# goldbricklemon/uplift-upsample-3dhpe

Hardware: AMD Instinct MI355X
Metric: pose-sequences/sec (higher is better)
Workload: dtype f16x3 (f32 operands split into f16 hi/lo, 3 MFMA passes, f32 accumulate); 1 GPU; config/h36m_351.json forward, N=71 tokens (receptive field 351), J=17, batch 128/GPU, s_in=5, seeded Keras-default weights; global_batch=128, parallelism=batch-sharded x1, hipgraph=True, concurrent_half_batches=False, batches_in_flight=8

## Files before the change

uplift-upsample-3dhpe_amd/csrc/uu3d_commit.inc:

```
namespace {

struct Packer {
    std::vector<float> buf;
    std::vector<std::pair<size_t, size_t>> dense;
    size_t alloc(size_t n) {
        size_t off = align_up(buf.size(), 64);
        buf.resize(off + n, 0.f);
        return off;
    }
    size_t alloc_dense(size_t n) { const size_t off = alloc(n); dense.emplace_back(off, n); return off; }
};

const float* W(const uu3d_model* m, const std::string& name) {
    auto it = m->index.find(name);
    return it == m->index.end() ? nullptr : m->weights[it->second].host.data();
}

void pack_dense_t(std::vector<float>& buf, size_t off, const float* w, int K, int N, int Kp, int n0) {
    for (int k = 0; k < K; ++k)
        for (int n = 0; n < N; ++n) buf[off + (size_t)(n0 + n) * Kp + k] = w[(size_t)k * N + n];
}

}

// ... 165 lines not shown
        };
        auto add_qkv = [&](TcBuild& tb, const std::string& p) {
            std::vector<float> Wk, b, bf; qkv_of(p, Wk, b);
            tb.stages.push_back(folded(Wk, b, W(m, p + "/norm1/gamma"), W(m, p + "/norm1/beta"), dt, 3 * dt, bf));
            for (int n = 0; n < dt; ++n) bf[n] *= tc_qscale;
            std::copy_n(bf.begin(), 3 * dt, P.buf.begin() + tb.p_off + TCP_BQKV);
        };
        auto add_proj = [&](TcBuild& tb, const std::string& p) {
            const float* w = W(m, p + "/attn/projection/kernel");
            tb.stages.push_back(TcStage{std::vector<float>(w, w + (size_t)dt * dt), dt, dt, 0, true});
            std::copy_n(W(m, p + "/attn/projection/bias"), dt, P.buf.begin() + tb.p_off + TCP_BP);
        };
        auto add_fc1 = [&](TcBuild& tb, const std::string& p) {
            const float* w = W(m, p + "/mlp/fc1/kernel"); const float* b = W(m, p + "/mlp/fc1/bias");
            std::vector<float> bf;
            tb.stages.push_back(folded(std::vector<float>(w, w + (size_t)dt * ht), std::vector<float>(b, b + ht), W(m, p + "/norm2/gamma"), W(m, p + "/norm2/beta"), dt, ht, bf));
            std::copy_n(bf.begin(), ht, P.buf.begin() + tb.p_off + TCP_B1);
        };
        auto add_fc2 = [&](TcBuild& tb, const std::string& p) {
            const float* w = W(m, p + "/mlp/fc2/kernel");
            for (int half = 0; half < 2; ++half) tb.stages.push_back(TcStage{std::vector<float>(w, w + (size_t)ht * dt), ht, dt, half * dt, false});
            std::copy_n(W(m, p + "/mlp/fc2/bias"), dt, P.buf.begin() + tb.p_off + TCP_B2);
        };
        { TcBuild tb{TC_QKV, P.alloc(TCP_FLOATS), {}}; add_qkv(tb, block_name(false, 0)); tcb.push_back(std::move(tb)); }
        for (int i = 0; i < c.temporal_depth; ++i) {
            const bool last = i + 1 == c.temporal_depth;
            TcBuild tb{TC_PROJ | TC_MLP | (last ? (c.num_strided > 0 ? TC_QKV | TC_PE : 0) : TC_QKV), P.alloc(TCP_FLOATS), {}};
            add_proj(tb, block_name(false, i)); add_fc1(tb, block_name(false, i)); add_fc2(tb, block_name(false, i));
            if (!last) add_qkv(tb, block_name(false, i + 1)); else if (c.num_strided > 0) add_qkv(tb, block_name(true, 0));
            tcb.push_back(std::move(tb));
        }
        if (c.num_strided > 0) {
            TcBuild tb{TC_PROJ | TC_FC1_PLANES, P.alloc(TCP_FLOATS), {}};
            add_proj(tb, block_name(true, 0)); add_fc1(tb, block_name(true, 0));
            tcb.push_back(std::move(tb));
        }
    }

    if (m->arena_floats < P.buf.size()) {
        if (m->arena) HIPCHK(m, hipFree(m->arena));
        m->arena = nullptr;
        HIPCHK(m, hipMalloc((void**)&m->arena, P.buf.size() * sizeof(float)));
        m->arena_floats = P.buf.size();
    }
    HIPCHK(m, hipMemcpyAsync(m->arena, P.buf.data(), P.buf.size() * sizeof(float), hipMemcpyHostToDevice, stream));
    HIPCHK(m, hipStreamSynchronize(stream));
    if (c.precision == UU3D_PREC_F16X3) {
        std::vector<_Float16> hb(64, (_Float16)0.f);
        m->hplanes.clear();
        for (auto& d : P.dense) {
            const size_t hi = align_up(hb.size(), 64); hb.resize(hi + d.second);
// ... 144 lines not shown
```

uplift-upsample-3dhpe_amd/csrc/uu3d_forward.inc:

```

namespace {
struct Workspace {
    float *S, *X, *QKV, *O, *Hb, *XA, *XB, *slab, *mslab;
    unsigned char* tc_scratch;
    int* frame_list;
    float2* stats;
    size_t slab_floats;
    size_t bytes;
};
Workspace carve(const uu3d_model* m, int B, char* base) {
    const uu3d_config& c = m->cfg;
    const size_t rows = (size_t)B * c.num_frames;
    const size_t rows_s = (size_t)B * (c.num_strided > 1 ? std::max(m->L[1], 1) : 1);
    size_t off = 0;
    auto take = [&](size_t n) { size_t o = off; off = align_up(off + n, 256); return o; };
    Workspace w{};
    const size_t oS = take(rows * c.num_keypoints * c.d_spatial * 4);
    const size_t oX = take(rows * c.d_temporal * 4);
    const size_t oQ = take((rows + 128) * 3 * c.d_temporal * 4);
    const size_t oO = take((rows + 32) * c.d_temporal * 4);
    const size_t oH = take((rows + 32) * c.h_temporal * 4);
    const size_t oA = take(rows * c.d_temporal * 4);
    const size_t oB = take(rows_s * c.d_temporal * 4);
    const size_t oT = take(rows * sizeof(float2));
// ... 243 lines not shown
            else gemm_tile<64, 64>(al, Bt, M, N, Kp, 1, KT, ep);
        } else {
            EpSlab es{slab, ldslab, (size_t)M * ldslab};
            gemm_tile<64, 64>(al, Bt, M, N, Kp, slices, kps, es);
            hipLaunchKernelGGL(splitk_reduce_kernel<EP>, dim3((M * N + 255) / 256), dim3(256), 0, stream,
                               slab, slices, (size_t)M * ldslab, M, N, ldslab, ep);
        }
        end();
    }

    bool mlpf_ok(int M, const BlockDev& b) const {
        return !m->sw.no_mlpf && b.w2_mf != 0 && panel_ok(M, m->cfg.h_temporal, m->cfg.d_temporal, b.w1_pf);
    }
    void mlp_fused(const char* name, const _Float16* Af, const BlockDev& b, int M, float* mslab) {
        if (skip_mask() & 8) return;
        const int mt = (M + 127) / 128, S = MLPF_SLICES;
        begin(name, "mlp_fused", 4.0 * M * (double)m->cfg.d_temporal * m->cfg.h_temporal, 4.0 * ((double)M * 384 + 2.0 * 384 * 768 + 3.0 * M * 384));
        allow_lds<mlp_fused_h3_kernel>(PANEL_LDS_TOTAL);
        hipLaunchKernelGGL(mlp_fused_h3_kernel, dim3(8 * S, ((mt * S + 7) / 8 + S - 1) / S), dim3(256), PANEL_LDS_TOTAL, stream,
                           Af, m->harena + b.w1_pf, m->harena + b.w2_mf, b.b1, mslab, M, mt);
        end();
    }
    void tchain(const char* name, const uu3d_model::TcLaunch& t, int M, const _Float16* Of, float* X, float* XA, const float* pe, int period,
                _Float16* Q, _Float16* H, unsigned char* scratch) {
        if (skip_mask() & 128) return;
        const int mt = (M + 63) / 64;
        TChainArgs a{};
        a.M = M; a.m_tiles = mt; a.period = period; a.qscale = attn_qscale();
        a.Of = Of; a.X = X; a.XA = XA; a.pe = pe; a.W = m->harena + t.w_off; a.P = m->arena + t.p_off; a.Q = Q; a.H = H; a.scratch = scratch;
        const double cols = ((t.flags & TC_PROJ) ? 384.0 : 0.0) + ((t.flags & TC_MLP) ? 1536.0 : 0.0) + ((t.flags & TC_FC1_PLANES) ? 768.0 : 0.0) + ((t.flags & TC_QKV) ? 1152.0 : 0.0);
        begin(name, "tchain", 2.0 * M * 384.0 * cols, 4.0 * (384.0 * cols + 2.0 * M * 384.0 + ((t.flags & TC_QKV) ? M * 1152.0 : 0.0) + ((t.flags & TC_FC1_PLANES) ? M * 768.0 : 0.0)));
#define UU3D_T16_LAUNCH(F) case F: { allow_lds<tchain16_kernel<F>>(T16_LDS_TOTAL); \
            hipLaunchKernelGGL(tchain16_kernel<F>, dim3(mt), dim3(512), T16_LDS_TOTAL, stream, a); } break;
        switch (t.flags) {
            UU3D_T16_LAUNCH(TC_QKV)
            UU3D_T16_LAUNCH(TC_PROJ | TC_MLP | TC_QKV)
            UU3D_T16_LAUNCH(TC_PROJ | TC_MLP | TC_QKV | TC_PE)
            UU3D_T16_LAUNCH(TC_PROJ | TC_MLP)
            UU3D_T16_LAUNCH(TC_PROJ | TC_FC1_PLANES)
            default: status = UU3D_ERR_UNSUPPORTED; m->err = "temporal chain: unknown stage set"; break;
        }
#undef UU3D_T16_LAUNCH
        end();
    }
    void ln_res_split_frag(const char* name, float* x, int M, const float* bias2, const float* mslab, float* xa, const float* pe, int period,
                           const float* g, const float* b, _Float16* Af) {
        if (skip_mask() & 64) return;
        begin(name, "ln_split_frag", 0.0, 4.0 * (double)M * 384 * (xa ? 8 : 7));
        hipLaunchKernelGGL((ln_res_split_frag_kernel<24, 8>), dim3((M + 7) / 8), dim3(128), 0, stream, x, 384, M, 1e-5f, bias2, mslab, xa, pe, period, g, b, Af);
        end();
    }

    bool wt_ok(const float* Bt, int K) const {
        return precision == UU3D_PREC_F16X3 && !m->sw.no_wt && (K % 16) == 0 && m->hplanes.count((size_t)(Bt - m->arena)) != 0;
    }
    template <class AL, class EP>
    void gemm_wt(const char* name, const AL& al, const float* Bt, int M, int N, int K, const EP& ep, double extra_bytes = 0) {
        const int Kp = round_up(K, 32), slices = Kp / 16;
        const auto it = m->hplanes.find((size_t)(Bt - m->arena));
        const _Float16* Bh = m->harena + it->second.first; const _Float16* Bl = m->harena + it->second.second;
        const int mt = (M + 31) / 32, nt = (N + 31) / 32;
// ... 125 lines not shown
constexpr int kFewRows = 512;

struct Forward {
    uu3d_model* const m;
    Launcher Lh;
    const Workspace w;
    const uu3d_config c;
    const uint8_t* const mask;
    const int B;
    float* const full_out; float* const central_out; float* const* const attn_out;
    const bool part_body, part_tail;

    const int N = c.num_frames, J = c.num_keypoints, dt = c.d_temporal, ht = c.h_temporal, M = B * N;
    const bool has_h1 = c.full_output && c.temporal_depth > 0;
    const bool planes = (c.precision == UU3D_PREC_F16X3) && (dt % 32 == 0) && (ht % 32 == 0) && !m->sw.no_planes;
    const bool chain = Lh.throughput && planes && m->sw.tchain_mode != 0 && (m->sw.tchain_mode == 1 || (M + 127) / 128 >= m->sw.tchain_min_tiles) && !m->tchain.empty() && M >= 1024 &&
                       (Lh.attn_is_h3(N, true) || (m->sw.tchain_short && Lh.attn_h3_any(N))) && (c.num_strided == 0 || m->L[0] == N) && (double)M * 1152 * 4.0 < 4.0e9 &&
                       attn_out == nullptr;
    _Float16* const Ph = reinterpret_cast<_Float16*>(w.O);
    _Float16* const Hh = reinterpret_cast<_Float16*>(w.Hb);
    const BlockDev* pend = nullptr;
    float* xa = w.XA;
    char nm[48];

    void tokens_from_frames(const FramesIn& frames) {
        Lh.begin("frames_to_tokens", "frames_to_tokens", 0.0, 4.0 * 3.0 * M * dt);
        hipLaunchKernelGGL(frames_to_tokens_kernel, dim3((unsigned)(((size_t)M * (dt / 4) + 255) / 256)), dim3(256), 0, Lh.stream,
                           frames.features, frames.num_rows, frames.rows, mask, m->token, m->pe_t, (long)M, N, dt, w.X);
        Lh.end();
    }
    void spatial(const float* kp2d) {
        spatial_stage(Lh, c, kp2d, M, mask, w.frame_list, w.S, true, EpSpatialToTemporal{w.X, m->s2t_b, dt, mask, m->token, m->pe_t, N});
    }

    const _Float16* block_head(const char* tag, int i, const BlockDev& b, float* x, int L, const uint8_t* kmask, const BlockDev* prev, bool fuse_mlp) {
        const int Mr = B * L;
        auto name = [&](const char* what) { snprintf(nm, sizeof nm, "%s%d.%s", tag, i + 1, what); return nm; };
        _Float16* const Pl = Ph + (size_t)Mr * dt; _Float16* const Hl = Hh + (size_t)Mr * ht;
        const bool qsplit = Lh.attn_is_h3(L, planes);
        _Float16* const Qh = reinterpret_cast<_Float16*>(w.QKV); _Float16* const Ql = Qh + (size_t)Mr * 3 * dt;
        const EpBiasSplitQ ep_qs{Qh, Ql, b.bqkv, 3 * dt, dt, Lh.attn_qscale()};
        const bool few = planes && Mr <= kFewRows && Lh.wt_ok(b.wqkv_t, dt) && Lh.wt_ok(b.w1_t, dt);
        auto maps = [&]() {
            if (attn_out != nullptr && tag[0] == 't' && attn_out[i] != nullptr) {
                Lh.begin(name("attn_maps"), "attn_probs", 2.0 * B * (double)c.num_heads * L * L * kDH, 4.0 * B * (double)c.num_heads * L * L);
                const size_t lds = (size_t)L * (kDH + 1) * sizeof(float);
// ... 43 lines not shown
        }
        if (mlp_panel) {
            if (!ln2_done) Lh.ln_split_frag(name("ln2_split"), x, Mr, b.ln2_g, b.ln2_b, Ph);
            if (fuse_mlp) return Ph;
            Lh.gemm_panel(name("ln_fc1"), Ph, b.w1_pf, b.b1, Mr, ht, PanelEpBiasReluSplit{Hh, Hl, ht});
        } else {
            Lh.row_stats(name("stats2"), x, dt, Mr, w.stats);
            ALoadLayerNorm al{x, w.stats, b.ln2_g, b.ln2_b, dt, Mr, dt};
            if (planes) { EpBiasReluSplit ep{Hh, Hl, b.b1, ht}; Lh.gemm(name("ln_fc1"), al, b.w1_t, Mr, ht, dt, ep); }
            else { EpBiasRelu ep{w.Hb, b.b1, ht}; Lh.gemm(name("ln_fc1"), al, b.w1_t, Mr, ht, dt, ep); }
        }
        return nullptr;
    }

    void temporal_chain() {
        _Float16* const Q = reinterpret_cast<_Float16*>(w.QKV);
        Lh.tchain("t1.ln_qkv", m->tchain[0], M, nullptr, w.X, nullptr, nullptr, 1, Q, nullptr, w.tc_scratch);
        for (int i = 0; i < c.temporal_depth; ++i) {
            const bool masked = c.has_strided_input && i < c.first_strided_token_attention_layer;
            snprintf(nm, sizeof nm, "t%d.attn", i + 1);
            Lh.attn(nm, w.QKV, B, N, masked ? mask : nullptr, w.O, (size_t)M * dt, true, true);
            const bool to_strided = i + 1 == c.temporal_depth && c.num_strided > 0;
            snprintf(nm, sizeof nm, "t%d.chain", i + 1);
            Lh.tchain(nm, m->tchain[i + 1], M, Ph, w.X, to_strided ? w.XA : nullptr, to_strided ? m->sblocks[0].pe : nullptr, N, Q, nullptr, w.tc_scratch);
        }
    }
    void temporal_blocks() {
        for (int i = 0; i < c.temporal_depth; ++i) {
            const BlockDev& b = m->tblocks[i];
            const bool masked = c.has_strided_input && i < c.first_strided_token_attention_layer;
            const bool last = (i + 1 == c.temporal_depth);
            const bool fuse = planes && Lh.mlpf_ok(M, b) && (last ? (c.num_strided > 0 && Lh.panel_ok(M, 3 * dt, dt, m->sblocks[0].wqkv_pf))
                                                                  : Lh.panel_ok(M, 3 * dt, dt, m->tblocks[i + 1].wqkv_pf));
            const _Float16* const a2 = block_head("t", i, b, w.X, N, masked ? mask : nullptr, pend, fuse);
            pend = nullptr;
            if (fuse) {
                snprintf(nm, sizeof nm, "t%d.mlp", i + 1);
                Lh.mlp_fused(nm, a2, b, M, w.mslab);
                pend = &b;
                continue;
            }
            const bool to_strided = last && c.num_strided > 0;
            EpBiasResidual ep_fc2{w.X, b.b2, dt, to_strided ? w.XA : nullptr, to_strided ? m->sblocks[0].pe : nullptr, N};
            snprintf(nm, sizeof nm, "t%d.fc2_res", i + 1);
            if (planes) { GLoadPlain gl{Hh, Hh + (size_t)M * ht, ht, M}; Lh.gemm_g(nm, gl, b.w2_t, M, dt, ht, ep_fc2, 4.0 * M * dt); }
            else { ALoadPlain al{w.Hb, ht, M, ht}; Lh.gemm(nm, al, b.w2_t, M, dt, ht, ep_fc2, 4.0 * M * dt); }
        }
    }
    void head1() {
        if (!has_h1) return;
        ALoadPlain al{w.X, dt, M, dt}; EpBias ep{full_out, m->h1_b, 3 * J};
        Lh.gemm("head1", al, m->h1_wt, M, 3 * J, dt, ep);
    }
    void strided_blocks() {
        float* xb = w.XB;
        const _Float16* const hzero = m->harena;
        if (c.temporal_depth == 0 && c.num_strided > 0) {
            Lh.begin("s1.add_pe", "add_pe", 0.0, 12.0 * M * dt);
            hipLaunchKernelGGL(add_period_kernel, dim3((unsigned)(((size_t)M * dt / 4 + 255) / 256)), dim3(256), 0, Lh.stream, w.X, m->sblocks[0].pe, M, dt, N, w.XA);
            Lh.end();
        }
        for (int i = 0; i < c.num_strided; ++i) {
            const BlockDev& b = m->sblocks[i];
            const int Li = m->L[i], Lo = m->L[i + 1], Mi = B * Li, Mo = B * Lo;
            if (((skip_mask() & 256) || part_body) && i >= 1) continue;
            if (((skip_mask() & 512) || part_tail) && i == 0) { std::swap(xa, xb); xb = w.XA; continue; }
            const int lo = (c.strides[i] > 1 && c.pad_left[i] == 0) ? 1 : 0;
            const EpConvResidual ep_conv{xb, b.b2, dt, xa, Li, Lo, c.strides[i], lo,
                                         (i + 1 < c.num_strided) ? m->sblocks[i + 1].pe : nullptr};
            const bool smask = c.temporal_depth == 0 && c.has_strided_input && i < c.first_strided_token_attention_layer;
            if (chain && i == 0) {
                Lh.attn("s1.attn", w.QKV, B, Li, nullptr, w.O, (size_t)Mi * dt, true, true);
                Lh.tchain("s1.chain", m->tchain[c.temporal_depth + 1], Mi, Ph, nullptr, xa, nullptr, 1, nullptr, Hh, w.tc_scratch);
            } else
            block_head("s", i, b, xa, Li, smask ? mask : nullptr, i == 0 ? pend : nullptr, false);
            if (i == 0) head1();
            snprintf(nm, sizeof nm, "s%d.conv_res", i + 1);
            if (planes) { GLoadConv3 gl{Hh, Hh + (size_t)Mi * ht, hzero, ht, Li, Lo, c.strides[i], c.pad_left[i], Mo};
                          Lh.gemm_g(nm, gl, b.w2_t, Mo, dt, 3 * ht, ep_conv, 4.0 * Mo * dt); }
            else { ALoadConv3 al{w.Hb, ht, Li, Lo, c.strides[i], c.pad_left[i], Mo, 3 * ht};
                   Lh.gemm(nm, al, b.w2_t, Mo, dt, 3 * ht, ep_conv, 4.0 * Mo * dt); }
            std::swap(xa, xb);
            if (i == 0) xb = w.XA;
        }
    }
    void head2() {
        ALoadPlain al{c.num_strided > 0 ? xa : w.X + (size_t)(N / 2) * dt, c.num_strided > 0 ? dt : N * dt, B, dt};
        EpBias ep{central_out, m->h2_b, 3 * J};
        Lh.gemm("head2", al, m->h2_wt, B, 3 * J, dt, ep);
    }
    void range_check() {
        if (c.precision != UU3D_PREC_F16X3) return;
        Lh.begin("range_check", "range_check", 0.0, 4.0 * ((has_h1 ? (double)M * 3 * J : 0.0) + (double)B * 3 * J));
        hipLaunchKernelGGL(range_check_kernel, dim3(256), dim3(256), 0, Lh.stream, has_h1 ? full_out : central_out, has_h1 ? (long)M * 3 * J : 0L,
                           central_out, (long)B * 3 * J, m->d_range);
        Lh.end();
    }
};

int forward_impl(uu3d_model* m, const float* kp2d, const FramesIn* frames, const uint8_t* mask, int32_t B, float* full_out,
                 float* central_out, float* const* attn_out, void* workspace, size_t workspace_bytes, int32_t schedule, void* stream_) {
    if (!m) return UU3D_ERR_INVALID_ARGUMENT;
    const bool exact_f32 = (schedule & UU3D_SCHEDULE_EXACT_F32) != 0;
    schedule &= ~UU3D_SCHEDULE_EXACT_F32;
#ifdef UU3D_TIMING_BUILD
    const bool parts_ok = process_switches().timing_parts;
#else
    constexpr bool parts_ok = false;
#endif
    const bool part_body = parts_ok && (schedule & 0x200) != 0, part_tail = parts_ok && (schedule & 0x400) != 0;
    if (parts_ok) schedule &= ~0x600;
    if (schedule != UU3D_SCHEDULE_LATENCY && schedule != UU3D_SCHEDULE_THROUGHPUT) return fail(m, UU3D_ERR_INVALID_ARGUMENT, "schedule must be UU3D_SCHEDULE_LATENCY or UU3D_SCHEDULE_THROUGHPUT");
    if (!m->committed) return fail(m, UU3D_ERR_NOT_READY, "uu3d_commit_weights has not been called");
    if ((!kp2d && !frames) || !central_out || !workspace || B < 1) return fail(m, UU3D_ERR_INVALID_ARGUMENT, "null buffer or batch < 1");
    if (frames != nullptr) {
// ... 106 lines not shown
```

uplift-upsample-3dhpe_amd/csrc/uu3d_gemm.h:

```cpp
#pragma once
#include "uu3d_dropout.h"
#include <hip/hip_runtime.h>
#include <stdint.h>

namespace uu3d {

typedef float f32x4 __attribute__((ext_vector_type(4)));
typedef float f32x16 __attribute__((ext_vector_type(16)));

static constexpr int GEMM_BK = 32;
static constexpr int GEMM_LD = 36;

__host__ __device__ inline constexpr size_t gemm_lds_bytes(int BM, int BN) {
    return (size_t)2 * (BM + BN) * GEMM_LD * sizeof(float);
}

struct ALoadPlain {
    const float* __restrict__ A;
    int lda, M, K;
    struct Ctx { const float* p; };
    struct Raw { f32x4 x; };
    __device__ __forceinline__ Ctx prep(int row) const {
        Ctx c; c.p = A + (size_t)min(row, M - 1) * lda; return c;
    }
// ... 50 lines not shown
    }
    __device__ __forceinline__ Raw issue(const Ctx& c, int k) const {
        const int kc = min(k, K - 4);
        const int j = kc / C;
        const int cc = kc - j * C;
        const int src = c.t0 + j;
        Raw r;
        r.ok = (src >= 0) & (src < L_in) & (k < K);
        const int srcc = min(max(src, 0), L_in - 1);
        r.x = *reinterpret_cast<const f32x4*>(Hin + (size_t)(c.base_row + srcc) * C + cc);
        return r;
    }
    __device__ __forceinline__ f32x4 finish(const Ctx&, int, const Raw& r) const {
        return r.ok ? r.x : (f32x4){0.f, 0.f, 0.f, 0.f};
    }
};

struct EpBias {
    float* __restrict__ out; const float* __restrict__ bias; int ldo;
    __device__ __forceinline__ float2 colv(int col) const { return make_float2(bias[col], 0.f); }
    __device__ __forceinline__ float2 pre(int, int) const { return make_float2(0.f, 0.f); }
    __device__ __forceinline__ void store(int row, int col, float v, float2 cv, float2) const {
        out[(size_t)row * ldo + col] = v + cv.x;
    }
};
struct EpBiasRelu {
    float* __restrict__ out; const float* __restrict__ bias; int ldo;
    __device__ __forceinline__ float2 colv(int col) const { return make_float2(bias[col], 0.f); }
    __device__ __forceinline__ float2 pre(int, int) const { return make_float2(0.f, 0.f); }
    __device__ __forceinline__ void store(int row, int col, float v, float2 cv, float2) const {
        out[(size_t)row * ldo + col] = fmaxf(v + cv.x, 0.f);
    }
};
struct EpBiasResidual {
    float* x; const float* __restrict__ bias; int ld;
    float* out2; const float* __restrict__ pe2; int period;
    __device__ __forceinline__ float2 colv(int col) const { return make_float2(bias[col], 0.f); }
    __device__ __forceinline__ float2 pre(int rowc, int col) const {
        float2 p; p.x = x[(size_t)rowc * ld + col];
        p.y = (out2 != nullptr) ? pe2[(size_t)(rowc % period) * ld + col] : 0.f;
        return p;
    }
    __device__ __forceinline__ void store(int row, int col, float v, float2 cv, float2 p) const {
        const size_t o = (size_t)row * ld + col;
        const float y = p.x + (v + cv.x);
        x[o] = y;
// ... 248 lines not shown
```

uplift-upsample-3dhpe_amd/csrc/uu3d_tchain16.h:

```cpp
#pragma once
#include <algorithm>
#include "uu3d_gemm_panel8.h"

namespace uu3d {

enum : int {
    TC_PROJ = 1,
    TC_MLP = 2,
    TC_QKV = 4,
    TC_FC1_PLANES = 8,
    TC_PE = 16,
};

static constexpr int TC_CHUNK_HALFS = P8_CHUNK_BYTES / 2;
__host__ __device__ inline constexpr int tchain_chunks(int flags) {
    return ((flags & TC_PROJ) ? 12 : 0) + ((flags & TC_MLP) ? 48 : 0) + ((flags & TC_FC1_PLANES) ? 24 : 0) + ((flags & TC_QKV) ? 36 : 0);
}
static constexpr size_t TC_TRASH_BYTES = 16384;

enum : int { TCP_BP = 0, TCP_B1 = 384, TCP_B2 = 1152, TCP_BQKV = 1536, TCP_FLOATS = 2688 };

struct TChainArgs {
    int M, m_tiles, period; float qscale;
    const _Float16* Of;
    float* X;
    float* XA; const float* pe;
    const _Float16* W;
    const float* P;
    _Float16* Q;
    _Float16* H;
    unsigned char* scratch;
};

__host__ __device__ inline size_t tchain_qf_index(size_t token, int ch, int plane) {
    const int u = ch >> 4, w = ch & 15, j = ((w >> 3) << 2) | (w & 3), g = (w >> 2) & 1;
    return ((((token >> 5) * 72 + u) * 2 + plane) * 64 + (token & 31) + 32 * g) * 8 + j;
}
__host__ __device__ inline constexpr size_t tchain_qf_halfs(int m_tiles) { return (size_t)m_tiles * 4 * 72 * 2 * 512; }

static constexpr size_t T16_X_FLOATS_PER_TILE = 64 * 384;
__host__ __device__ inline constexpr size_t tchain16_scratch_bytes(int m_tiles64) {
    return (size_t)m_tiles64 * (2 * T16_X_FLOATS_PER_TILE * 4) + TC_TRASH_BYTES;
}
inline void tchain16_reorder_mlp(const _Float16* in, _Float16* out) {
    const size_t C = TC_CHUNK_HALFS;
    std::copy(in, in + 12 * C, out);
    std::copy(in + 24 * C, in + 36 * C, out + 12 * C);
    std::copy(in + 12 * C, in + 24 * C, out + 24 * C);
    std::copy(in + 36 * C, in + 48 * C, out + 36 * C);
}

static constexpr size_t T16_XCHG_BYTES = 8 * 1024;
static constexpr size_t T16_BIAS_BYTES = 1152 * 4;
static constexpr size_t T16_LDS_TOTAL = P8_RING_BYTES + T16_XCHG_BYTES + T16_BIAS_BYTES;
// ... 2 lines not shown
    const int tile = row >> 6, q = (row >> 4) & 3, t = row & 15;
    const int c = ch >> 5, hh = (ch >> 4) & 1, g = (ch >> 2) & 3, r = ch & 3;
    return (size_t)tile * T16_X_FLOATS_PER_TILE + (((size_t)(c * 8 + 4 * hh + q) * 64 + t + 16 * g) * 4 + r);
}

inline void tchain16_pack_stage(const _Float16* Bh, const _Float16* Bl, int N, int Kp, int kofs, bool natural, _Float16* out) {
    for (int c = 0; c < N / 32; ++c)
        for (int hh = 0; hh < 2; ++hh)
            for (int kk = 0; kk < 12; ++kk)
                for (int p = 0; p < 2; ++p)
                    for (int l = 0; l < 64; ++l)
                        for (int j = 0; j < 8; ++j) {
                            const int S = kk >> 1, mm = kk & 1, t = l & 15, g = l >> 4;
                            const int n = 32 * c + 16 * (mm ^ hh) + t;
                            const int k = natural ? 16 * (12 * hh + 2 * S + (g >> 1)) + 8 * (j >> 2) + 4 * (g & 1) + (j & 3)
                                                  : kofs + 32 * (2 * S + (j >> 2)) + 16 * hh + 4 * g + (j & 3);
                            out[(((((size_t)c * 2 + hh) * 12 + kk) * 2 + p) * 64 + l) * 8 + j] = (p ? Bl : Bh)[(size_t)n * Kp + k];
                        }
}

template <bool BIAS> struct T16EpResidual { static constexpr int kStores = 0; static constexpr bool kBias = BIAS; const float* bias; int nbias; };
struct T16EpHidden { static constexpr int kStores = 0; static constexpr bool kBias = true; const float* bias; int nbias; };
struct T16EpQkv { static constexpr int kStores = 2; static constexpr bool kBias = true; h16x4* __restrict__ qf; const float* bias; int nbias; };
struct T16EpPlanes { static constexpr int kStores = 2; static constexpr bool kBias = true; unsigned char* __restrict__ ph; unsigned char* __restrict__ pl; const float* bias; int nbias; };

#ifndef UU3D_T16_DEPTH
#define UU3D_T16_DEPTH 2
#endif
#ifndef UU3D_T16_LOO
#define UU3D_T16_LOO 0
#endif

template <int FLAGS>
__global__ void __launch_bounds__(512) __attribute__((amdgpu_waves_per_eu(2, 2)))
tchain16_kernel(const TChainArgs a)
{
    constexpr int HS = 12, KS = 6;
    constexpr int GT = tchain_chunks(FLAGS);
    static_assert(!((FLAGS & TC_MLP) && (FLAGS & TC_FC1_PLANES)), "one MLP form per launch");
    static_assert(GT >= 12, "at least one stage");
    h3_flush_f16_denormals();
    extern __shared__ __attribute__((aligned(16))) unsigned char psm[];

    const int bm = blockIdx.x;
    const int tid = threadIdx.x, lane = tid & 63, wave = __builtin_amdgcn_readfirstlane(tid >> 6);
    const int hh = wave >> 2, q = wave & 3, g = lane >> 4, t = lane & 15;
    const int tok = bm * 64 + q * 16 + t;
    const bool live = tok < a.M;
    const int tokc = min(tok, a.M - 1);
    const int chl = 16 * hh + 4 * g;

    const unsigned wofs = (unsigned)(hh * HS * 2048 + q * 3072);
    const unsigned char* const wsrc = reinterpret_cast<const unsigned char*>(a.W) + wofs;
    const unsigned lane16 = (unsigned)lane * 16u;
    auto dma1 = [&](int Gc, int j, int slot, int i) __attribute__((always_inline)) {
        if (UU3D_T16_LOO & 1) return;
        const unsigned char* s = wsrc + (size_t)min(Gc, GT - 1) * P8_CHUNK_BYTES + j * (6 * 2048);
        unsigned char* d = psm + slot * P8_CHUNK_BYTES + wofs + j * (6 * 2048);
        switch (i) {
            case 0: __builtin_amdgcn_global_load_lds((h3_glb_void*)(s + lane16), (h3_lds_void*)d, 16, 0, 0); break;
            case 1: __builtin_amdgcn_global_load_lds((h3_glb_void*)(s + lane16), (h3_lds_void*)d, 16, 1024, 0); break;
            default: __builtin_amdgcn_global_load_lds((h3_glb_void*)(s + lane16), (h3_lds_void*)d, 16, 2048, 0); break;
        }
    };

    f32x4 xr[12];
    h16x8 ah[KS], al[KS];
    h16x8 fh[KS], fl[KS];
    constexpr int DP = UU3D_T16_DEPTH, RB = DP + 1;
    h16x8 bh[RB] = {}, bl[RB] = {};

    auto late = [&](int v) __attribute__((always_inline)) -> int { asm volatile("" : "+s"(v)); return v; };
    const unsigned xoff = (unsigned)(wave * 256 + lane * 4);
    auto xs_tile = [&](int b, bool strided1) __attribute__((always_inline)) -> float* {
        return reinterpret_cast<float*>(a.scratch) + ((size_t)b + (strided1 ? (size_t)a.m_tiles : 0)) * T16_X_FLOATS_PER_TILE;
    };
    auto load_xs = [&](const float* tl) __attribute__((always_inline)) {
#pragma unroll
        for (int c = 0; c < 12; ++c) xr[c] = *reinterpret_cast<const f32x4*>(tl + (xoff + (unsigned)(c * 2048)));
    };
    auto store_xs = [&](float* tl) __attribute__((always_inline)) {
        unsigned xo = xoff;
        asm volatile("" : "+v"(xo));
#pragma unroll
        for (int c = 0; c < 12; ++c) *reinterpret_cast<f32x4*>(tl + (xo + (unsigned)(c * 2048))) = xr[c];
    };
    auto load_rows = [&](const float* base) __attribute__((always_inline)) {
        const float* p = base + (size_t)tokc * 384 + chl;
#pragma unroll
        for (int c = 0; c < 12; ++c) xr[c] = *reinterpret_cast<const f32x4*>(p + 32 * c);
    };
    auto store_rows = [&](float* base) __attribute__((always_inline)) {
        const int tk = late(bm) * 64 + q * 16 + t;
// ... 25 lines not shown
    unsigned char* const xmine = psm + P8_RING_BYTES + wave * 1024 + lane16;
    unsigned char* const xpart = psm + P8_RING_BYTES + (wave ^ 4) * 1024 + lane16;
    float* const stat = reinterpret_cast<float*>(psm + P8_RING_BYTES);
    float* const bias_lds = reinterpret_cast<float*>(psm + P8_RING_BYTES + T16_XCHG_BYTES);
    const unsigned rd0 = (unsigned)(uintptr_t)(h3_lds_void*)(psm + hh * HS * 2048 + lane16);
    const unsigned bias_rd = (unsigned)(uintptr_t)(h3_lds_void*)(psm + P8_RING_BYTES + T16_XCHG_BYTES) + (unsigned)chl * 4u;

#define UU3D_T16_READ(i, sb, kk) \
    asm volatile("ds_read_b128 %0, %2 offset:%3\n\tds_read_b128 %1, %2 offset:%4" \
                 : "=&v"(bh[i]), "=&v"(bl[i]) : "v"(sb), "i"((kk) * 2048), "i"((kk) * 2048 + 1024))

    struct Acc { f32x4 a0[2], a1[2]; };
    struct Fin { f32x4 u, s, r, b, y; h16x4 vh, vl; };
    struct Keep { h16x4 h, l; };
    using I0 = std::integral_constant<int, 0>; using I1 = std::integral_constant<int, 1>; using I2 = std::integral_constant<int, 2>; using I3 = std::integral_constant<int, 3>;

    auto fin_a = [&](auto ep, auto fin_tag, const int j, Fin& f) __attribute__((always_inline)) {
        using EP = decltype(ep);
        constexpr int fs = decltype(fin_tag)::value;
        float y = f.u[j] + f.r[j];
        if constexpr (EP::kBias) y += f.b[j];
        if constexpr (std::is_same<EP, T16EpResidual<false>>::value || std::is_same<EP, T16EpResidual<true>>::value) {
            xr[fs][j] += y;
        } else {
            if constexpr (std::is_same<EP, T16EpHidden>::value || std::is_same<EP, T16EpPlanes>::value) y = fmaxf(y, 0.f);
            _Float16 h; float hf;
            asm("v_cvt_f16_f32 %0, %2\n\tv_cvt_f32_f16 %1, %0" : "=&v"(h), "=v"(hf) : "v"(y));
            f.y[j] = y - hf;
            f.vh[j] = h;
        }
    };
    auto fin_b = [&](auto ep, const int j, Fin& f) __attribute__((always_inline)) {
        using EP = decltype(ep);
        if constexpr (!(std::is_same<EP, T16EpResidual<false>>::value || std::is_same<EP, T16EpResidual<true>>::value))
            f.vl[j] = (_Float16)(f.y[j] * H3_SCALE);
    };
    auto fin_store = [&](auto ep, const int cp, auto fin_tag, Fin& f, Keep& hk) __attribute__((always_inline)) {
        using EP = decltype(ep);
        constexpr int fs = decltype(fin_tag)::value;
        if constexpr (std::is_same<EP, T16EpHidden>::value) {
            if constexpr ((fs & 1) == 0) { hk.h = f.vh; hk.l = f.vl; }
            else {
                h16x8 ph, pl;
#pragma unroll
                for (int e = 0; e < 4; ++e) { ph[e] = hk.h[e]; ph[4 + e] = f.vh[e]; pl[e] = hk.l[e]; pl[4 + e] = f.vl[e]; }
                constexpr int ks = fs == 11 ? 5 : fs >> 1;
                fh[ks] = ph; fl[ks] = pl;
            }
        } else if constexpr (std::is_same<EP, T16EpQkv>::value) {
            h16x4* d = ep.qf + (size_t)(2 * cp + hh) * 256;
            d[0] = f.vh; d[128] = f.vl;
        } else if constexpr (std::is_same<EP, T16EpPlanes>::value) {
            const unsigned o = (unsigned)(32 * cp) * 2u;
            *reinterpret_cast<h16x4*>(ep.ph + o) = f.vh;
            *reinterpret_cast<h16x4*>(ep.pl + o) = f.vl;
        }
    };

    auto chunk = [&](auto cl_tag, auto pre_tag, const int c, auto fin_tag, auto ep, const h16x8 (&Ah)[KS], const h16x8 (&Al)[KS],
                     Acc& x, const Acc& p, Keep& hk, const int bias_c0) __attribute__((always_inline)) {
        constexpr int CL = decltype(cl_tag)::value;
        constexpr bool PRE_IN = (decltype(pre_tag)::value & 1) != 0, PRE_OUT = (decltype(pre_tag)::value & 2) != 0;
        using EP = decltype(ep);
        constexpr int NST = EP::kStores;
        constexpr bool FIN = CL > 0 && !(UU3D_T16_LOO & 2);
        const int pslot = slot == 0 ? 2 : slot - 1;
        const unsigned sb = rd0 + (unsigned)slot * P8_CHUNK_BYTES;
        Fin f;
        auto gapwork = [&](const int gp) __attribute__((always_inline)) {
            if constexpr (CL > 0 && (UU3D_T16_LOO & 2) != 0) { if (gp == 3) asm volatile("" :: "v"(p.a0[0]), "v"(p.a0[1]), "v"(p.a1[0]), "v"(p.a1[1])); }
            if constexpr (FIN) {
                if (gp == 3 || gp == 4) {
#pragma unroll
                    for (int e = 0; e < 2; ++e) { const int k = 2 * (gp - 3) + e; f.s[k] = p.a0[1][k] + p.a1[1][k] * (1.0f / H3_SCALE); }
                }
                if (gp == 5) asm volatile("ds_write_b128 %0, %1" :: "v"((unsigned)(uintptr_t)(h3_lds_void*)xmine), "v"(f.s) : "memory");
                if (gp >= 9 && gp <= 12) f.u[gp - 9] = p.a0[0][gp - 9] + p.a1[0][gp - 9] * (1.0f / H3_SCALE);
                if (gp >= 22 && gp <= 25) fin_b(ep, gp - 22, f);
// ... 63 lines not shown
    auto stage_tail = [&](auto ep, const int c, auto fin_tag, const Acc& p, Keep& hk, const int bias_c0) __attribute__((always_inline)) {
        using EP = decltype(ep);
        asm volatile("s_waitcnt vmcnt(0) lgkmcnt(0)" ::: "memory");
        __builtin_amdgcn_s_barrier();
        Fin f;
#pragma unroll
        for (int e = 0; e < 4; ++e) { f.s[e] = p.a0[1][e] + p.a1[1][e] * (1.0f / H3_SCALE); f.u[e] = p.a0[0][e] + p.a1[0][e] * (1.0f / H3_SCALE); }
        asm volatile("ds_write_b128 %0, %1\n\ts_waitcnt lgkmcnt(0)" :: "v"((unsigned)(uintptr_t)(h3_lds_void*)xmine), "v"(f.s) : "memory");
        __builtin_amdgcn_s_barrier();
        asm volatile("ds_read_b128 %0, %1" : "=&v"(f.r) : "v"((unsigned)(uintptr_t)(h3_lds_void*)xpart) : "memory");
        if constexpr (EP::kBias) asm volatile("ds_read_b128 %0, %1" : "=&v"(f.b) : "v"(bias_rd + (unsigned)(bias_c0 + c) * 128u) : "memory");
        else f.b = f32x4{0.f, 0.f, 0.f, 0.f};
        asm volatile("s_waitcnt lgkmcnt(0)" : "+v"(f.r), "+v"(f.b));
#pragma unroll
        for (int j = 0; j < 4; ++j) { fin_a(ep, fin_tag, j, f); fin_b(ep, j, f); }
        fin_store(ep, c, fin_tag, f, hk);
        __builtin_amdgcn_s_barrier();
    };

    using F0 = std::integral_constant<int, 0>; using F1 = std::integral_constant<int, 1>; using F2 = std::integral_constant<int, 2>; using F11 = std::integral_constant<int, 11>;
    auto stage = [&](auto nch_tag, auto ep, const h16x8 (&Ah)[KS], const h16x8 (&Al)[KS], const int bias_c0) __attribute__((always_inline)) {
        constexpr int NCH = decltype(nch_tag)::value;
        using EP = decltype(ep);
        static_assert(NCH % 4 == 0 && NCH >= 8, "bodies of four chunks");
        if constexpr (EP::kBias) {
            for (int i = tid; i < ep.nbias / 4; i += 512) reinterpret_cast<f32x4*>(bias_lds)[i] = reinterpret_cast<const f32x4*>(ep.bias)[i];
        }
        auto rotate = [&]() __attribute__((always_inline)) {
            if constexpr (std::is_same<EP, T16EpResidual<false>>::value || std::is_same<EP, T16EpResidual<true>>::value) {
                static_assert(NCH == 12, "three rotations");
#pragma unroll
                for (int s = 0; s < 4; ++s) { const f32x4 tt = xr[s]; xr[s] = xr[s + 4]; xr[s + 4] = xr[s + 8]; xr[s + 8] = tt; __builtin_amdgcn_sched_barrier(0); }
            } else if constexpr (std::is_same<EP, T16EpHidden>::value) {
                static_assert(NCH == 12, "three rotations");
#pragma unroll
                for (int s = 0; s < 2; ++s) {
                    const h16x8 th = fh[s], tl = fl[s];
                    fh[s] = fh[s + 2]; fl[s] = fl[s + 2]; fh[s + 2] = fh[s + 4]; fl[s + 2] = fl[s + 4]; fh[s + 4] = th; fl[s + 4] = tl;
                    __builtin_amdgcn_sched_barrier(0);
                }
            }
        };
        Acc xa, xb;
#pragma unroll
        for (int m = 0; m < 2; ++m) { xb.a0[m] = f32x4{0.f, 0.f, 0.f, 0.f}; xb.a1[m] = f32x4{0.f, 0.f, 0.f, 0.f}; }
        Keep hk{};
        chunk(I0{}, I2{}, 0, F0{}, ep, Ah, Al, xa, xb, hk, bias_c0);
        chunk(I1{}, I3{}, 1, F0{}, ep, Ah, Al, xb, xa, hk, bias_c0);
        chunk(I2{}, I3{}, 2, F1{}, ep, Ah, Al, xa, xb, hk, bias_c0);
        chunk(I3{}, I1{}, 3, F2{}, ep, Ah, Al, xb, xa, hk, bias_c0);
        rotate();
#pragma unroll 1
        for (int c = 4; c < NCH; c += 4) {
            chunk(I3{}, I2{}, c, F11{}, ep, Ah, Al, xa, xb, hk, bias_c0);
            chunk(I3{}, I3{}, c + 1, F0{}, ep, Ah, Al, xb, xa, hk, bias_c0);
            chunk(I3{}, I3{}, c + 2, F1{}, ep, Ah, Al, xa, xb, hk, bias_c0);
            chunk(I3{}, I1{}, c + 3, F2{}, ep, Ah, Al, xb, xa, hk, bias_c0);
            rotate();
        }
        stage_tail(ep, (int)(NCH - 1), F11{}, xb, hk, bias_c0);
    };
    using N12 = std::integral_constant<int, 12>;

    auto token_sum = [&](float s, int phase) __attribute__((always_inline)) -> float {
        s += __shfl_xor(s, 16);
        s += __shfl_xor(s, 32);
        if (g == 0) stat[phase * 128 + wave * 16 + t] = s;
        asm volatile("s_waitcnt lgkmcnt(0)" ::: "memory");
        __builtin_amdgcn_s_barrier();
        asm volatile("" ::: "memory");
        return s + stat[phase * 128 + (wave ^ 4) * 16 + t];
    };
    auto layer_norm = [&]() __attribute__((always_inline)) {
        float s = 0.f;
#pragma unroll
        for (int c = 0; c < 12; ++c) s += (xr[c][0] + xr[c][1]) + (xr[c][2] + xr[c][3]);
        const float mean = token_sum(s, 0) * (1.0f / 384.0f);
        float v = 0.f;
#pragma unroll
        for (int c = 0; c < 12; ++c) {
            const f32x4 d = xr[c] - mean;
            v += (d[0] * d[0] + d[1] * d[1]) + (d[2] * d[2] + d[3] * d[3]);
        }
// ... 6 lines not shown
#pragma unroll
            for (int e = 0; e < 4; ++e) { ah[S][e] = hi[0][e]; ah[S][4 + e] = hi[1][e]; al[S][e] = lo[0][e]; al[S][4 + e] = lo[1][e]; }
        }
    };

    if constexpr ((FLAGS & TC_PROJ) != 0) {
        stage(N12{}, T16EpResidual<true>{a.P + TCP_BP, 384}, ah, al, 0);
        if constexpr (kStrided1) store_rows(a.XA);
    } else {
        store_xs(xs_tile(bm, false));
    }
    if constexpr ((FLAGS & (TC_MLP | TC_FC1_PLANES)) != 0) {
        layer_norm();
        if constexpr (kStrided1) {
            unsigned char* const trash = a.scratch + (size_t)a.m_tiles * (2 * T16_X_FLOATS_PER_TILE * 4);
            unsigned char* ph = live ? reinterpret_cast<unsigned char*>(a.H + (size_t)tok * 768 + chl) : trash;
            unsigned char* pl = live ? reinterpret_cast<unsigned char*>(a.H + ((size_t)a.M + tok) * 768 + chl) : trash + 4096;
            stage(std::integral_constant<int, 24>{}, T16EpPlanes{ph, pl, a.P + TCP_B1, 768}, ah, al, 0);
        } else {
            stage(N12{}, T16EpHidden{a.P + TCP_B1, 384}, ah, al, 0);
            stage(N12{}, T16EpResidual<false>{nullptr, 0}, fh, fl, 0);
            stage(N12{}, T16EpHidden{a.P + TCP_B1 + 384, 384}, ah, al, 0);
            stage(N12{}, T16EpResidual<true>{a.P + TCP_B2, 384}, fh, fl, 0);
            if constexpr ((FLAGS & TC_QKV) == 0 || (FLAGS & TC_PE) != 0) store_rows(a.X);
        }
    }
    if constexpr ((FLAGS & TC_QKV) != 0) {
        if constexpr ((FLAGS & TC_PE) != 0) {
            const int tkc = min(late(bm) * 64 + q * 16 + t, a.M - 1);
            const float* pr = a.pe + (size_t)(tkc % a.period) * 384 + chl;
#pragma unroll
            for (int c = 0; c < 12; ++c) xr[c] = xr[c] + *reinterpret_cast<const f32x4*>(pr + 32 * c);
            store_xs(xs_tile(late(bm), true));
        } else if constexpr ((FLAGS & (TC_PROJ | TC_MLP)) != 0) {
            store_xs(xs_tile(late(bm), false));
        }
        layer_norm();
        const int lb = late(bm);
        h16x4* const qf = reinterpret_cast<h16x4*>(a.Q) + ((size_t)(lb * 2 + (q >> 1)) * (72 * 2 * 64) + (q & 1) * 16 + t + 32 * (g & 1)) * 2 + (g >> 1);
        stage(std::integral_constant<int, 36>{}, T16EpQkv{qf, a.P + TCP_BQKV, 1152}, ah, al, 0);
    }
    asm volatile("s_waitcnt vmcnt(0)" ::: "memory");
#undef UU3D_T16_READ
}

}
```

Measured before the change: 205,100 pose-sequences/s.

## Fuse head1 projection and range check into final temporal chain kernel

Adds a two-chunk head1 stage to the last temporal chain kernel. It computes the 51-wide full-sequence output directly from the register-resident activations, writes it out, and flags non-finite values. When head1 is fused this also skips the X row store for the strided path, and head2 gets a range-checking epilogue, so the separate head1 GEMM and range_check launches go away. The cost is a heavier, more register-hungry chain kernel, extra template instantiations, and atomics in the epilogues.

```diff
diff --git a/uplift-upsample-3dhpe_amd/csrc/uu3d_commit.inc b/uplift-upsample-3dhpe_amd/csrc/uu3d_commit.inc
--- a/uplift-upsample-3dhpe_amd/csrc/uu3d_commit.inc
+++ b/uplift-upsample-3dhpe_amd/csrc/uu3d_commit.inc
@@ -211,11 +211,21 @@
             for (int half = 0; half < 2; ++half) tb.stages.push_back(TcStage{std::vector<float>(w, w + (size_t)ht * dt), ht, dt, half * dt, false});
             std::copy_n(W(m, p + "/mlp/fc2/bias"), dt, P.buf.begin() + tb.p_off + TCP_B2);
         };
+        auto add_head1 = [&](TcBuild& tb) {
+            const int Nn = 32 * TC_H1_CHUNKS;
+            TcStage st{std::vector<float>((size_t)dt * Nn, 0.f), dt, Nn, 0, false};
+            for (int n = 0; n < 3 * J; ++n) for (int k = 0; k < dt; ++k) st.Wk[(size_t)k * Nn + n] = P.buf[o_h1 + (size_t)n * Kdt + k];
+            tb.stages.push_back(std::move(st));
+            std::copy_n(P.buf.begin() + o_h1b, 3 * J, P.buf.begin() + tb.p_off + TCP_BH1);
+        };
         { TcBuild tb{TC_QKV, P.alloc(TCP_FLOATS), {}}; add_qkv(tb, block_name(false, 0)); tcb.push_back(std::move(tb)); }
         for (int i = 0; i < c.temporal_depth; ++i) {
             const bool last = i + 1 == c.temporal_depth;
-            TcBuild tb{TC_PROJ | TC_MLP | (last ? (c.num_strided > 0 ? TC_QKV | TC_PE : 0) : TC_QKV), P.alloc(TCP_FLOATS), {}};
+            static_assert(3 * kJ == TC_H1_OUT, "head1's row length is compiled into the chain (non-generic handles have J = kJ)");
+            const bool h1 = last && has_h1;
+            TcBuild tb{TC_PROJ | TC_MLP | (h1 ? TC_HEAD1 : 0) | (last ? (c.num_strided > 0 ? TC_QKV | TC_PE : 0) : TC_QKV), P.alloc(TCP_FLOATS), {}};
             add_proj(tb, block_name(false, i)); add_fc1(tb, block_name(false, i)); add_fc2(tb, block_name(false, i));
+            if (h1) add_head1(tb);
             if (!last) add_qkv(tb, block_name(false, i + 1)); else if (c.num_strided > 0) add_qkv(tb, block_name(true, 0));
             tcb.push_back(std::move(tb));
         }
diff --git a/uplift-upsample-3dhpe_amd/csrc/uu3d_forward.inc b/uplift-upsample-3dhpe_amd/csrc/uu3d_forward.inc
--- a/uplift-upsample-3dhpe_amd/csrc/uu3d_forward.inc
+++ b/uplift-upsample-3dhpe_amd/csrc/uu3d_forward.inc
@@ -289,21 +289,26 @@
         end();
     }
     void tchain(const char* name, const uu3d_model::TcLaunch& t, int M, const _Float16* Of, float* X, float* XA, const float* pe, int period,
-                _Float16* Q, _Float16* H, unsigned char* scratch) {
+                _Float16* Q, _Float16* H, unsigned char* scratch, float* full = nullptr) {
         if (skip_mask() & 128) return;
         const int mt = (M + 63) / 64;
         TChainArgs a{};
         a.M = M; a.m_tiles = mt; a.period = period; a.qscale = attn_qscale();
         a.Of = Of; a.X = X; a.XA = XA; a.pe = pe; a.W = m->harena + t.w_off; a.P = m->arena + t.p_off; a.Q = Q; a.H = H; a.scratch = scratch;
-        const double cols = ((t.flags & TC_PROJ) ? 384.0 : 0.0) + ((t.flags & TC_MLP) ? 1536.0 : 0.0) + ((t.flags & TC_FC1_PLANES) ? 768.0 : 0.0) + ((t.flags & TC_QKV) ? 1152.0 : 0.0);
-        begin(name, "tchain", 2.0 * M * 384.0 * cols, 4.0 * (384.0 * cols + 2.0 * M * 384.0 + ((t.flags & TC_QKV) ? M * 1152.0 : 0.0) + ((t.flags & TC_FC1_PLANES) ? M * 768.0 : 0.0)));
+        a.full = full; a.range = m->d_range;
+        if ((t.flags & TC_HEAD1) && full == nullptr) { status = UU3D_ERR_INVALID_ARGUMENT; m->err = "temporal chain: head1 without full_out"; return; }
+        const bool h1 = (t.flags & TC_HEAD1) != 0, x_rows = !(h1 && (t.flags & TC_PE));
+        const double cols = (h1 ? (double)TC_H1_OUT : 0.0) + ((t.flags & TC_PROJ) ? 384.0 : 0.0) + ((t.flags & TC_MLP) ? 1536.0 : 0.0) + ((t.flags & TC_FC1_PLANES) ? 768.0 : 0.0) + ((t.flags & TC_QKV) ? 1152.0 : 0.0);
+        begin(name, "tchain", 2.0 * M * 384.0 * cols, 4.0 * (384.0 * cols + (x_rows ? 2.0 : 1.0) * M * 384.0 + (h1 ? (double)M * TC_H1_OUT : 0.0) + ((t.flags & TC_QKV) ? M * 1152.0 : 0.0) + ((t.flags & TC_FC1_PLANES) ? M * 768.0 : 0.0)));
 #define UU3D_T16_LAUNCH(F) case F: { allow_lds<tchain16_kernel<F>>(T16_LDS_TOTAL); \
             hipLaunchKernelGGL(tchain16_kernel<F>, dim3(mt), dim3(512), T16_LDS_TOTAL, stream, a); } break;
         switch (t.flags) {
             UU3D_T16_LAUNCH(TC_QKV)
             UU3D_T16_LAUNCH(TC_PROJ | TC_MLP | TC_QKV)
             UU3D_T16_LAUNCH(TC_PROJ | TC_MLP | TC_QKV | TC_PE)
+            UU3D_T16_LAUNCH(TC_PROJ | TC_MLP | TC_HEAD1 | TC_QKV | TC_PE)
             UU3D_T16_LAUNCH(TC_PROJ | TC_MLP)
+            UU3D_T16_LAUNCH(TC_PROJ | TC_MLP | TC_HEAD1)
             UU3D_T16_LAUNCH(TC_PROJ | TC_FC1_PLANES)
             default: status = UU3D_ERR_UNSUPPORTED; m->err = "temporal chain: unknown stage set"; break;
         }
@@ -475,6 +480,7 @@
     const BlockDev* pend = nullptr;
     float* xa = w.XA;
     char nm[48];
+    bool h1_in_chain() const { return chain && has_h1 && (m->tchain[c.temporal_depth].flags & TC_HEAD1) != 0; }
 
     void tokens_from_frames(const FramesIn& frames) {
         Lh.begin("frames_to_tokens", "frames_to_tokens", 0.0, 4.0 * 3.0 * M * dt);
@@ -564,7 +570,8 @@
             Lh.attn(nm, w.QKV, B, N, masked ? mask : nullptr, w.O, (size_t)M * dt, true, true);
             const bool to_strided = i + 1 == c.temporal_depth && c.num_strided > 0;
             snprintf(nm, sizeof nm, "t%d.chain", i + 1);
-            Lh.tchain(nm, m->tchain[i + 1], M, Ph, w.X, to_strided ? w.XA : nullptr, to_strided ? m->sblocks[0].pe : nullptr, N, Q, nullptr, w.tc_scratch);
+            Lh.tchain(nm, m->tchain[i + 1], M, Ph, w.X, to_strided ? w.XA : nullptr, to_strided ? m->sblocks[0].pe : nullptr, N, Q, nullptr, w.tc_scratch,
+                      (m->tchain[i + 1].flags & TC_HEAD1) ? full_out : nullptr);
         }
     }
     void temporal_blocks() {
@@ -590,7 +597,7 @@
         }
     }
     void head1() {
-        if (!has_h1) return;
+        if (!has_h1 || h1_in_chain()) return;
         ALoadPlain al{w.X, dt, M, dt}; EpBias ep{full_out, m->h1_b, 3 * J};
         Lh.gemm("head1", al, m->h1_wt, M, 3 * J, dt, ep);
     }
@@ -628,11 +635,12 @@
     }
     void head2() {
         ALoadPlain al{c.num_strided > 0 ? xa : w.X + (size_t)(N / 2) * dt, c.num_strided > 0 ? dt : N * dt, B, dt};
-        EpBias ep{central_out, m->h2_b, 3 * J};
-        Lh.gemm("head2", al, m->h2_wt, B, 3 * J, dt, ep);
-    }
+        if (range_folded()) Lh.gemm("head2", al, m->h2_wt, B, 3 * J, dt, EpBiasRange{central_out, m->h2_b, 3 * J, m->d_range});
+        else Lh.gemm("head2", al, m->h2_wt, B, 3 * J, dt, EpBias{central_out, m->h2_b, 3 * J});
+    }
+    bool range_folded() const { return c.precision == UU3D_PREC_F16X3 && chain && (!has_h1 || h1_in_chain()); }
     void range_check() {
-        if (c.precision != UU3D_PREC_F16X3) return;
+        if (c.precision != UU3D_PREC_F16X3 || range_folded()) return;
         Lh.begin("range_check", "range_check", 0.0, 4.0 * ((has_h1 ? (double)M * 3 * J : 0.0) + (double)B * 3 * J));
         hipLaunchKernelGGL(range_check_kernel, dim3(256), dim3(256), 0, Lh.stream, has_h1 ? full_out : central_out, has_h1 ? (long)M * 3 * J : 0L,
                            central_out, (long)B * 3 * J, m->d_range);
diff --git a/uplift-upsample-3dhpe_amd/csrc/uu3d_gemm.h b/uplift-upsample-3dhpe_amd/csrc/uu3d_gemm.h
--- a/uplift-upsample-3dhpe_amd/csrc/uu3d_gemm.h
+++ b/uplift-upsample-3dhpe_amd/csrc/uu3d_gemm.h
@@ -96,6 +96,16 @@
     __device__ __forceinline__ float2 pre(int, int) const { return make_float2(0.f, 0.f); }
     __device__ __forceinline__ void store(int row, int col, float v, float2 cv, float2) const {
         out[(size_t)row * ldo + col] = v + cv.x;
+    }
+};
+struct EpBiasRange {
+    float* __restrict__ out; const float* __restrict__ bias; int ldo; int* __restrict__ flag;
+    __device__ __forceinline__ float2 colv(int col) const { return make_float2(bias[col], 0.f); }
+    __device__ __forceinline__ float2 pre(int, int) const { return make_float2(0.f, 0.f); }
+    __device__ __forceinline__ void store(int row, int col, float v, float2 cv, float2) const {
+        const float y = v + cv.x;
+        out[(size_t)row * ldo + col] = y;
+        if (!(fabsf(y) <= 3.0e38f)) atomicOr(flag, 1);
     }
 };
 struct EpBiasRelu {
diff --git a/uplift-upsample-3dhpe_amd/csrc/uu3d_tchain16.h b/uplift-upsample-3dhpe_amd/csrc/uu3d_tchain16.h
--- a/uplift-upsample-3dhpe_amd/csrc/uu3d_tchain16.h
+++ b/uplift-upsample-3dhpe_amd/csrc/uu3d_tchain16.h
@@ -10,15 +10,18 @@
     TC_QKV = 4,
     TC_FC1_PLANES = 8,
     TC_PE = 16,
+    TC_HEAD1 = 32,
 };
+static constexpr int TC_H1_OUT = 51, TC_H1_CHUNKS = 2;
 
 static constexpr int TC_CHUNK_HALFS = P8_CHUNK_BYTES / 2;
 __host__ __device__ inline constexpr int tchain_chunks(int flags) {
-    return ((flags & TC_PROJ) ? 12 : 0) + ((flags & TC_MLP) ? 48 : 0) + ((flags & TC_FC1_PLANES) ? 24 : 0) + ((flags & TC_QKV) ? 36 : 0);
+    return ((flags & TC_PROJ) ? 12 : 0) + ((flags & TC_MLP) ? 48 : 0) + ((flags & TC_FC1_PLANES) ? 24 : 0) + ((flags & TC_QKV) ? 36 : 0) +
+           ((flags & TC_HEAD1) ? TC_H1_CHUNKS : 0);
 }
 static constexpr size_t TC_TRASH_BYTES = 16384;
 
-enum : int { TCP_BP = 0, TCP_B1 = 384, TCP_B2 = 1152, TCP_BQKV = 1536, TCP_FLOATS = 2688 };
+enum : int { TCP_BP = 0, TCP_B1 = 384, TCP_B2 = 1152, TCP_BQKV = 1536, TCP_BH1 = 2688, TCP_FLOATS = 2752 };
 
 struct TChainArgs {
     int M, m_tiles, period; float qscale;
@@ -30,6 +33,8 @@
     _Float16* Q;
     _Float16* H;
     unsigned char* scratch;
+    float* full;
+    int* range;
 };
 
 __host__ __device__ inline size_t tchain_qf_index(size_t token, int ch, int plane) {
@@ -78,6 +83,7 @@
 template <bool BIAS> struct T16EpResidual { static constexpr int kStores = 0; static constexpr bool kBias = BIAS; const float* bias; int nbias; };
 struct T16EpHidden { static constexpr int kStores = 0; static constexpr bool kBias = true; const float* bias; int nbias; };
 struct T16EpQkv { static constexpr int kStores = 2; static constexpr bool kBias = true; h16x4* __restrict__ qf; const float* bias; int nbias; };
+struct T16EpHead1 { static constexpr int kStores = 4; static constexpr bool kBias = true; float* __restrict__ out; float* __restrict__ trash; int lim; const float* bias; int nbias; };
 struct T16EpPlanes { static constexpr int kStores = 2; static constexpr bool kBias = true; unsigned char* __restrict__ ph; unsigned char* __restrict__ pl; const float* bias; int nbias; };
 
 #ifndef UU3D_T16_DEPTH
@@ -95,6 +101,7 @@
     constexpr int GT = tchain_chunks(FLAGS);
     static_assert(!((FLAGS & TC_MLP) && (FLAGS & TC_FC1_PLANES)), "one MLP form per launch");
     static_assert(GT >= 12, "at least one stage");
+    static_assert(!(FLAGS & TC_HEAD1) || (FLAGS & TC_MLP), "head1 reads the finished temporal stack");
     h3_flush_f16_denormals();
     extern __shared__ __attribute__((aligned(16))) unsigned char psm[];
 
@@ -125,6 +132,7 @@
     h16x8 fh[KS], fl[KS];
     constexpr int DP = UU3D_T16_DEPTH, RB = DP + 1;
     h16x8 bh[RB] = {}, bl[RB] = {};
+    unsigned h1_bad = 0;
 
     auto late = [&](int v) __attribute__((always_inline)) -> int { asm volatile("" : "+s"(v)); return v; };
     const unsigned xoff = (unsigned)(wave * 256 + lane * 4);
@@ -196,6 +204,8 @@
         if constexpr (EP::kBias) y += f.b[j];
         if constexpr (std::is_same<EP, T16EpResidual<false>>::value || std::is_same<EP, T16EpResidual<true>>::value) {
             xr[fs][j] += y;
+        } else if constexpr (std::is_same<EP, T16EpHead1>::value) {
+            f.y[j] = y;
         } else {
             if constexpr (std::is_same<EP, T16EpHidden>::value || std::is_same<EP, T16EpPlanes>::value) y = fmaxf(y, 0.f);
             _Float16 h; float hf;
@@ -206,7 +216,7 @@
     };
     auto fin_b = [&](auto ep, const int j, Fin& f) __attribute__((always_inline)) {
         using EP = decltype(ep);
-        if constexpr (!(std::is_same<EP, T16EpResidual<false>>::value || std::is_same<EP, T16EpResidual<true>>::value))
+        if constexpr (!(std::is_same<EP, T16EpResidual<false>>::value || std::is_same<EP, T16EpResidual<true>>::value || std::is_same<EP, T16EpHead1>::value))
             f.vl[j] = (_Float16)(f.y[j] * H3_SCALE);
     };
     auto fin_store = [&](auto ep, const int cp, auto fin_tag, Fin& f, Keep& hk) __attribute__((always_inline)) {
@@ -228,6 +238,14 @@
             const unsigned o = (unsigned)(32 * cp) * 2u;
             *reinterpret_cast<h16x4*>(ep.ph + o) = f.vh;
             *reinterpret_cast<h16x4*>(ep.pl + o) = f.vl;
+        } else if constexpr (std::is_same<EP, T16EpHead1>::value) {
+#pragma unroll
+            for (int r = 0; r < 4; ++r) {
+                const bool ok = 32 * cp + r < ep.lim;
+                float* const d = ok ? ep.out + (32 * cp + r) : ep.trash + r;
+                *d = f.y[r];
+                h1_bad |= (ok && !(fabsf(f.y[r]) <= 3.0e38f)) ? 1u : 0u;
+            }
         }
     };
 
@@ -337,7 +355,7 @@
     auto stage = [&](auto nch_tag, auto ep, const h16x8 (&Ah)[KS], const h16x8 (&Al)[KS], const int bias_c0) __attribute__((always_inline)) {
         constexpr int NCH = decltype(nch_tag)::value;
         using EP = decltype(ep);
-        static_assert(NCH % 4 == 0 && NCH >= 8, "bodies of four chunks");
+        static_assert((NCH % 4 == 0 && NCH >= 8) || NCH == 2, "bodies of four chunks, or the two-chunk form");
         if constexpr (EP::kBias) {
             for (int i = tid; i < ep.nbias / 4; i += 512) reinterpret_cast<f32x4*>(bias_lds)[i] = reinterpret_cast<const f32x4*>(ep.bias)[i];
         }
@@ -360,20 +378,27 @@
 #pragma unroll
         for (int m = 0; m < 2; ++m) { xb.a0[m] = f32x4{0.f, 0.f, 0.f, 0.f}; xb.a1[m] = f32x4{0.f, 0.f, 0.f, 0.f}; }
         Keep hk{};
-        chunk(I0{}, I2{}, 0, F0{}, ep, Ah, Al, xa, xb, hk, bias_c0);
-        chunk(I1{}, I3{}, 1, F0{}, ep, Ah, Al, xb, xa, hk, bias_c0);
-        chunk(I2{}, I3{}, 2, F1{}, ep, Ah, Al, xa, xb, hk, bias_c0);
-        chunk(I3{}, I1{}, 3, F2{}, ep, Ah, Al, xb, xa, hk, bias_c0);
-        rotate();
+        if constexpr (NCH == 2) {
+            static_assert(std::is_same<EP, T16EpHead1>::value, "the two-chunk form has no register rotation");
+            chunk(I0{}, I2{}, 0, F0{}, ep, Ah, Al, xa, xb, hk, bias_c0);
+            chunk(I1{}, I1{}, 1, F0{}, ep, Ah, Al, xb, xa, hk, bias_c0);
+            stage_tail(ep, 1, F1{}, xb, hk, bias_c0);
+        } else {
+            chunk(I0{}, I2{}, 0, F0{}, ep, Ah, Al, xa, xb, hk, bias_c0);
+            chunk(I1{}, I3{}, 1, F0{}, ep, Ah, Al, xb, xa, hk, bias_c0);
+            chunk(I2{}, I3{}, 2, F1{}, ep, Ah, Al, xa, xb, hk, bias_c0);
+            chunk(I3{}, I1{}, 3, F2{}, ep, Ah, Al, xb, xa, hk, bias_c0);
+            rotate();
 #pragma unroll 1
-        for (int c = 4; c < NCH; c += 4) {
-            chunk(I3{}, I2{}, c, F11{}, ep, Ah, Al, xa, xb, hk, bias_c0);
-            chunk(I3{}, I3{}, c + 1, F0{}, ep, Ah, Al, xb, xa, hk, bias_c0);
-            chunk(I3{}, I3{}, c + 2, F1{}, ep, Ah, Al, xa, xb, hk, bias_c0);
-            chunk(I3{}, I1{}, c + 3, F2{}, ep, Ah, Al, xb, xa, hk, bias_c0);
-            rotate();
-        }
-        stage_tail(ep, (int)(NCH - 1), F11{}, xb, hk, bias_c0);
+            for (int c = 4; c < NCH; c += 4) {
+                chunk(I3{}, I2{}, c, F11{}, ep, Ah, Al, xa, xb, hk, bias_c0);
+                chunk(I3{}, I3{}, c + 1, F0{}, ep, Ah, Al, xb, xa, hk, bias_c0);
+                chunk(I3{}, I3{}, c + 2, F1{}, ep, Ah, Al, xa, xb, hk, bias_c0);
+                chunk(I3{}, I1{}, c + 3, F2{}, ep, Ah, Al, xb, xa, hk, bias_c0);
+                rotate();
+            }
+            stage_tail(ep, (int)(NCH - 1), F11{}, xb, hk, bias_c0);
+        }
     };
     using N12 = std::integral_constant<int, 12>;
 
@@ -426,7 +451,22 @@
             stage(N12{}, T16EpResidual<false>{nullptr, 0}, fh, fl, 0);
             stage(N12{}, T16EpHidden{a.P + TCP_B1 + 384, 384}, ah, al, 0);
             stage(N12{}, T16EpResidual<true>{a.P + TCP_B2, 384}, fh, fl, 0);
-            if constexpr ((FLAGS & TC_QKV) == 0 || (FLAGS & TC_PE) != 0) store_rows(a.X);
+            if constexpr ((FLAGS & TC_HEAD1) != 0) {
+#pragma unroll
+                for (int S = 0; S < KS; ++S) {
+                    h16x4 hi[2], lo[2];
+#pragma unroll
+                    for (int i = 0; i < 2; ++i) h3_split(xr[2 * S + i], hi[i], lo[i]);
+#pragma unroll
+                    for (int e = 0; e < 4; ++e) { ah[S][e] = hi[0][e]; ah[S][4 + e] = hi[1][e]; al[S][e] = lo[0][e]; al[S][4 + e] = lo[1][e]; }
+                }
+                const int tk = late(bm) * 64 + q * 16 + t;
+                float* const tr = reinterpret_cast<float*>(a.scratch + (size_t)a.m_tiles * (2 * T16_X_FLOATS_PER_TILE * 4)) + chl;
+                const bool lv = tk < a.M;
+                stage(std::integral_constant<int, TC_H1_CHUNKS>{}, T16EpHead1{lv ? a.full + (size_t)tk * TC_H1_OUT + chl : tr, tr, lv ? TC_H1_OUT - chl : 0, a.P + TCP_BH1, 32 * TC_H1_CHUNKS}, ah, al, 0);
+                if (__any((int)h1_bad) && lane == 0) atomicOr(a.range, 1);
+            }
+            if constexpr (((FLAGS & TC_QKV) == 0 || (FLAGS & TC_PE) != 0) && (FLAGS & (TC_HEAD1 | TC_PE)) != (TC_HEAD1 | TC_PE)) store_rows(a.X);
         }
     }
     if constexpr ((FLAGS & TC_QKV) != 0) {
```

Measured after the change: 208,400 pose-sequences/s, median of 6. 1.02x the previous value.
